# ZhengkunTian/OpenTransformer

Measured on AMD Instinct MI355X. Metric: utterances/sec (80-d fbank, ~1000 frames) train fwd+bwd, higher is better.
Workload: dtype fp16; 1 GPU; AISHELL-1 transformer_baseline.yaml (+input_size 80), 12 enc / 6 dec layers, B=32/GPU x 1000 frames x 80-d fbank, 15 decoder rows, V=4234, residual_dropout 0.1; step = fwd + bwd + grad all-reduce + clip/Adam/Noam; global_batch=32, frames=1000, parallelism=dp1, hipgraph=True

## Files before the change

include/otrans_hip.h:

```cpp
#ifndef OTRANS_HIP_H
#define OTRANS_HIP_H
#include <stddef.h>
#include <stdint.h>
#ifdef __cplusplus
extern "C" {
#endif

#define OTR_F32 0
#define OTR_BF16 1
#define OTR_F16 2
#define OTR_ACT_NONE 0
#define OTR_ACT_RELU 1

#define OTR_ABI_VERSION 604
int32_t otr_version(void);
int32_t otr_half_type(void);
int32_t otr_debug_set(int32_t key, int32_t value);
int32_t otr_set_fault_counter(void* device_word);
int32_t otr_debug_trread(const void* image, const int32_t* addr, void* out, void* stream);
int32_t otr_debug_trace(void* buf);
const char* otr_last_error_string(void);

typedef struct {
  int32_t M, N, K;
  int32_t x_dtype, w_dtype, y_dtype, compute;
  int64_t ldx, ldw, ldy;
  int32_t act;
  int32_t accumulate;
} otr_linear_desc_t;
int32_t otr_linear_fwd(const otr_linear_desc_t* d, const void* x, const void* w, const float* bias, void* y,
                       void* workspace, int64_t workspace_bytes, void* stream);
int32_t otr_linear_fwd_batched(const otr_linear_desc_t* d, const void* x, const void* w, void* y, int32_t nbatch, int64_t bsx, int64_t bsw,
                               int64_t bsy, void* stream);
int32_t otr_linear_dgrad(const otr_linear_desc_t* d, const void* dy, const void* w, void* dx, void* workspace,
                         int64_t workspace_bytes, void* stream);
int32_t otr_linear_wgrad(const otr_linear_desc_t* d, const void* dy, const void* x, void* dw, void* workspace,
                         int64_t workspace_bytes, void* stream);
int32_t otr_colsum(const void* a, int32_t dtype, int64_t M, int64_t N, int64_t lda, float* out, int32_t accumulate,
                   void* stream);

int32_t otr_ffn_glu_fwd(const void* x, int64_t ldx, const void* w1, int64_t ldw, const float* b1, void* h, void* u, int32_t M,
                        int32_t F, int32_t d_model, void* stream);
int32_t otr_ffn_glu_bwd(const void* dy, int32_t dy_dtype, int64_t ldy, const void* w2t, int64_t ldw, const void* h,
                        int32_t h_has_sigmoid, void* dh, float* dbias_partial, int32_t partial_rows_cap,
                        int32_t* partial_rows, int32_t M, int32_t F, int32_t d_model, void* stream);

int32_t otr_pack_frags(const void* src, void* dst, const int64_t* table, int32_t n_items, int64_t total_blocks,
// ... 221 lines not shown
int32_t otr_dwconv_bwd_part(const float* dy, const void* g, int32_t dtype, const float* w, void* dg, float* part, int32_t B, int32_t T,
                            int32_t C, int32_t k, int32_t pad, void* stream);
int32_t otr_bn_swish_fwd(const float* y, const float* stats, const float* gamma, const float* beta, float* running_mean,
                         float* running_var, float* saved, void* out, int32_t out_dtype, int64_t M, int32_t C, float eps,
                         float momentum, int32_t training, void* stream);
int64_t otr_dwconv_fwd_partial_rows(int64_t M);
int32_t otr_dwconv_fwd_part(const void* g, int32_t dtype, const float* w, const float* bias, float* y, float* spart, int32_t B, int32_t T,
                            int32_t C, int32_t k, int32_t pad, void* stream);
int32_t otr_bn_swish_fwd_part(const float* y, const float* spart, int32_t nblk, const float* gamma, const float* beta, float* running_mean,
                              float* running_var, float* saved, void* out, int32_t out_dtype, int64_t M, int32_t C, float eps,
                              float momentum, void* stream);
int32_t otr_bn_swish_bwd_partial_rows(int64_t M);
int32_t otr_bn_swish_bwd(const float* y, const void* ds, int32_t ds_dtype, const float* saved, const float* gamma,
                         const float* beta, float* red, float* partial, float* dgamma_acc, float* dbeta_acc, float* dy,
                         int64_t M, int32_t C, int32_t training, void* stream);
int32_t otr_bn_swish_bwd_sums(const float* y, const void* ds, int32_t ds_dtype, const float* saved, const float* gamma, const float* beta,
                              float* red, float* partial, float* dgamma_acc, float* dbeta_acc, int64_t M, int32_t C, void* stream);
int32_t otr_conformer_conv_bwd_mid(const float* y, const void* ds, const float* saved, const float* gamma, const float* beta,
                                   const float* red, const void* g, const float* w, const void* h, const uint8_t* row_mask, void* dh,
                                   float* part, float* gpart, int32_t dtype, int32_t training, int32_t B, int32_t T, int32_t C, int32_t k,
                                   int32_t pad, void* stream);

int32_t otr_ctc_loss(const float* log_probs, const int64_t* targets, int64_t ldt, const int32_t* in_len,
                     const int32_t* tgt_len, int32_t B, int32_t T, int32_t V, int32_t max_tgt, int32_t blank,
                     float* alpha_ws, float* nll, float* loss, float* dlogits, void* stream);

#define OTR_OPT_STATE_FLOATS 528
int32_t otr_optimizer_step(float* param, const float* grad, float* exp_avg, float* exp_avg_sq, int64_t n,
                           float* state, int32_t state_floats ,
                           void* param_bf16 ,
                           float base_lr, float beta1, float beta2, float eps, float weight_decay,
                           float grad_scale, float clip_norm, float noam_model_size, float noam_warmup,
                           float noam_factor, float noam_step_offset, float grad_noise_std, void* stream);

int32_t otr_allreduce_unique_id(void* id128);
int32_t otr_allreduce_init(void** handle, const void* id128, int32_t rank, int32_t world);
int32_t otr_allreduce_run(void* handle, void* buf, int64_t count, int32_t dtype, void* stream);
int32_t otr_allreduce_destroy(void* handle);

int32_t otr_beam_topk(const float* logits, int64_t ld, const float* lm_logits, int64_t ld_lm, float lm_weight,
                      int64_t rows, int32_t V, int32_t k, float* out_score, int64_t* out_idx, void* stream);
int32_t otr_beam_prune(const float* k_score, const int64_t* k_idx, const float* scores_in, const uint8_t* flag_in,
                       const int64_t* preds_in, int64_t ldp, int32_t batch, int32_t beam, int32_t t, int32_t eos,
                       float* scores_out, uint8_t* flag_out, int64_t* preds_out, int32_t* n_finished, void* stream);

int64_t otr_ctc_beam_workspace_bytes(int32_t B, int32_t T, int32_t W);
int32_t otr_ctc_topk(const float* log_probs, int64_t ld, const int32_t* lengths, int32_t B, int32_t T, int32_t V, int32_t K,
                     float* top_lp, int32_t* top_tok, void* stream);
int32_t otr_ctc_beam_search(const float* top_lp, const int32_t* top_tok, const int32_t* lengths, int32_t B, int32_t T, int32_t V,
                            int32_t K, int32_t blank, int32_t W, void* workspace, int64_t ws_bytes, int64_t* tokens,
                            int32_t* out_len, float* scores, void* stream);

int32_t otr_ngram_lookup(const void* table, int64_t capacity, int32_t max_probe, int32_t order, int32_t V, const int32_t* ctx,
                         const int32_t* ctx_len, const int32_t* tok, int64_t n, float oov_score, float* out, void* stream);
int32_t otr_ctc_beam_search_lm(const float* top_lp, const int32_t* top_tok, const int32_t* lengths, int32_t B, int32_t T, int32_t V,
                               int32_t K, int32_t blank, int32_t W, void* workspace, int64_t ws_bytes, int64_t* tokens,
                               int32_t* out_len, float* scores, const void* table, int64_t capacity, int32_t max_probe,
                               int32_t order, float alpha, float beta, float oov_score, float* lm_scores, void* stream);

int64_t otr_ctc_align_workspace_bytes(int32_t B, int32_t T, int32_t max_tgt);
int32_t otr_ctc_align(const float* log_probs, int64_t ld, const int64_t* targets, int64_t ldt, const int32_t* in_len,
                      const int32_t* tgt_len, int32_t B, int32_t T, int32_t V, int32_t max_tgt, int32_t blank, void* workspace,
                      int64_t ws_bytes, int32_t* frame_token, int32_t* spans, float* label_logp, float* score, void* stream);

int32_t otr_joint_prebeam(const float* logits, int64_t ld, const float* lm_logits, int64_t ld_lm, float att_weight, float lm_weight,
                          int64_t rows, int32_t V, int32_t K, float* cand_score, int32_t* cand_idx, void* stream);
// ... 111 lines not shown
```

opentransformer_amd/_lib.py:

```python
import ctypes as C
import os

_HERE = os.path.dirname(os.path.abspath(__file__))
_LIB_DIR = os.environ.get('OTR_LIB_DIR') or os.path.join(_HERE, 'lib')
LIB_PATHS = {'bf16': os.path.join(_LIB_DIR, 'libotrans_hip.so'), 'fp16': os.path.join(_LIB_DIR, 'libotrans_hip_f16.so')}
LIB_PATH = LIB_PATHS['bf16']

OTR_F32, OTR_BF16, OTR_F16 = 0, 1, 2
OTR_ABI_VERSION = 604
OTR_OPT_STATE_FLOATS = 528
ACT_NONE, ACT_RELU = 0, 1


class LinearDesc(C.Structure):
    _fields_ = [('M', C.c_int32), ('N', C.c_int32), ('K', C.c_int32),
                ('x_dtype', C.c_int32), ('w_dtype', C.c_int32), ('y_dtype', C.c_int32), ('compute', C.c_int32),
                ('ldx', C.c_int64), ('ldw', C.c_int64), ('ldy', C.c_int64),
                ('act', C.c_int32), ('accumulate', C.c_int32)]


class WgradItem(C.Structure):
    _fields_ = [('dy', C.c_void_p), ('x', C.c_void_p), ('dw', C.c_void_p), ('M', C.c_int32), ('N', C.c_int32),
                ('K', C.c_int32), ('ldy', C.c_int64), ('ldx', C.c_int64), ('ldw', C.c_int64),
                ('dy_dtype', C.c_int32), ('x_dtype', C.c_int32), ('dbias', C.c_void_p), ('overwrite', C.c_int32)]


class ColsumItem(C.Structure):
    _fields_ = [('a', C.c_void_p), ('out', C.c_void_p), ('M', C.c_int64), ('N', C.c_int64), ('lda', C.c_int64),
                ('dtype', C.c_int32)]


class AttnDesc(C.Structure):
    _fields_ = [('B', C.c_int32), ('H', C.c_int32), ('Tq', C.c_int32), ('Tk', C.c_int32), ('dk', C.c_int32),
                ('dtype', C.c_int32),
                ('q_bs', C.c_int64), ('q_ts', C.c_int64), ('k_bs', C.c_int64), ('k_ts', C.c_int64),
                ('v_bs', C.c_int64), ('v_ts', C.c_int64), ('o_bs', C.c_int64), ('o_ts', C.c_int64),
                ('causal', C.c_int32), ('scale', C.c_float)]


class LnDesc(C.Structure):
    _fields_ = [('M', C.c_int64), ('d', C.c_int32), ('a_dtype', C.c_int32),
                ('eps', C.c_float), ('p_drop', C.c_float), ('rng_offset', C.c_uint64), ('a_scale', C.c_float), ('a_row_mask', C.c_void_p),
# ... 111 lines not shown
    'otr_conv2_dgrad_wide': [C.POINTER(ConvDesc), _P, _P, _P, _P, _P, _I64, _P],
    'otr_debug_conv2_dgrad_plan': [C.POINTER(ConvDesc), _P],
    'otr_conv2_wgrad': [C.POINTER(ConvDesc), _P, _P, _P, _P, _I64, _P],
    'otr_relu_bwd': [_P, _P, _P, _I32, _I64, _P],
    'otr_relu_bwd_colsum_partial_rows': [_I64, _I32, _I32],
    'otr_relu_bwd_colsum': [_P, _P, _P, _P, _I32, _I64, _I32, _P],
    'otr_act_fwd': [_P, _P, _I32, _I64, _I32, _P],
    'otr_act_bwd': [_P, _P, _P, _I32, _I64, _I32, _P],
    'otr_label_smoothing_loss': [_P, _P, _I64, _I32, _F32, _I32, _P, _P, _P, _P],
    'otr_label_smoothing_loss_ld': [_P, _I64, _P, _I64, _I32, _F32, _I32, _P, _P, _I64, _P, _P],
    'otr_label_smoothing_loss_fused': [_P, _I64, _P, _I64, _I32, _I64, _I32, _F32, _I32, _P, _P, _P, _I32, _I64, _P, _P, _P],
    'otr_log_softmax': [_P, _P, _I64, _I32, _P],
    'otr_ctc_loss': [_P, _P, _I64, _P, _P, _I32, _I32, _I32, _I32, _I32, _P, _P, _P, _P, _P],
    'otr_ffn_fwd_split_slab': [_P, _P, _P, _P, _P, _P, _P, _I64, _I32, _I32, _P],
    'otr_ffn_bwd_split_slab': [_P, _P, _P, _P, _P, _P, _I64, _I32, _I32, _P],
    'otr_ln_bwd_proj_slabs': [_P, _P, _I32, _P, _P, _P, _P, _P, _P, _P, _P, _P, _I64, _P, _I64, _I32, _F32, C.c_uint64, _P],
    'otr_rb_linear_ln': [C.POINTER(DecLn), _P, _P, _P, _I32, _I64, _I64, _I32, _I32, _P],
    'otr_dec_self_fwd': [C.POINTER(DecLn), _I32, _I32, _P, _P, _P, _P, _P, _P, _P, _P],
    'otr_dec_self_step': [C.POINTER(DecLn), _I64, _P, _P, _P, _P, _P, _P, _P, _I32, _P, _P],
    'otr_dec_cross_fwd': [C.POINTER(DecLn), _I32, _I32, _P, _P, _P, _P, _I64, _I64, _I32, _I32, _P, _I32, _P, _P, _P, _P, _P],
    'otr_dec_cross_fwd_shared': [C.POINTER(DecLn), _I32, _I32, _P, _P, _P, _P, _I64, _I64, _I32, _I32, _P, _I32, _I32, _P, _P, _P, _P, _P],
    'otr_dec_ffn_hsave_bytes': [_I64, _I32],
    'otr_dec_ffn_fwd': [C.POINTER(DecLn), _I64, _P, _P, _P, _I32, _I32, _P, _P, _P],
    'otr_dec_ln': [C.POINTER(DecLn), _I64, _P],
    'otr_dec_self_step_pair': [C.POINTER(DecSelfStep), C.POINTER(DecSelfStep), _P],
    'otr_dec_ffn_fwd_pair': [C.POINTER(DecFfnFwd), C.POINTER(DecFfnFwd), _P],
    'otr_dec_ln_pair': [C.POINTER(DecLn), _I64, C.POINTER(DecLn), _I64, _P],
    'otr_dec_ffn_bwd': [C.POINTER(DecLnB), _I64, _P, _P, _P, _I32, _I32, _P, _P, _P, _P, _P],
    'otr_dec_cross_bwd': [C.POINTER(DecLnB), _I32, _I32, _P, _P, _P, _P, _P, _P, _P, _I64, _I64, _I32, _I32, _P, _I32, _P, _P, _P],
    'otr_dec_self_bwd': [C.POINTER(DecLnB), _I32, _I32, _P, _P, _P, _P, _P, _P, _P, _P],
    'otr_dec_sum': [_P, _P, _I32, _I64, _P, _P],
    'otr_dec_group_size': [_I32, _I32],
    'otr_optimizer_step': [_P, _P, _P, _P, _I64, _P, _I32, _P] + [_F32] * 12 + [_P],
    'otr_allreduce_unique_id': [_P],
    'otr_allreduce_init': [C.POINTER(C.c_void_p), _P, _I32, _I32],
    'otr_allreduce_run': [_P, _P, _I64, _I32, _P],
    'otr_allreduce_destroy': [_P],
    'otr_beam_topk': [_P, _I64, _P, _I64, _F32, _I64, _I32, _I32, _P, _P, _P],
    'otr_beam_prune': [_P, _P, _P, _P, _P, _I64, _I32, _I32, _I32, _I32, _P, _P, _P, _P, _P],
    'otr_beam_prune_cached': [_P, _P, _P, _P, _P, _I64, _I32, _I32, _I32, _P, _P, _P, _P, _I32, _P, _P, _P, _P, _P],
    'otr_ctc_beam_workspace_bytes': [_I32, _I32, _I32],
    'otr_ctc_topk': [_P, _I64, _P, _I32, _I32, _I32, _I32, _P, _P, _P],
    'otr_ctc_beam_search': [_P, _P, _P, _I32, _I32, _I32, _I32, _I32, _I32, _P, _I64, _P, _P, _P, _P],
    'otr_ngram_lookup': [_P, _I64, _I32, _I32, _I32, _P, _P, _P, _I64, _F32, _P, _P],
    'otr_ctc_beam_search_lm': [_P, _P, _P, _I32, _I32, _I32, _I32, _I32, _I32, _P, _I64, _P, _P, _P, _P, _I64, _I32, _I32, _F32, _F32,
                               _F32, _P, _P],
    'otr_ctc_align_workspace_bytes': [_I32, _I32, _I32],
    'otr_ctc_align': [_P, _I64, _P, _I64, _P, _P, _I32, _I32, _I32, _I32, _I32, _P, _I64, _P, _P, _P, _P, _P],
    'otr_joint_prebeam': [_P, _I64, _P, _I64, _F32, _F32, _I64, _I32, _I32, _P, _P, _P],
    'otr_ctc_prefix_score': [_P, _I64, _P, _I32, _I32, _I32, _I32, _I32, _I64, _I32, _I32, _P, _P, _P, _P, _I64, _I32, _P, _P, _P, _P, _P,
                             _F32, _P, _P, _P, _I32, _P, _P, _P, _P],
    'otr_beam_prune_joint': [_P, _P, _P, _P, _P, _I64, _I32, _I32, _I32, _I32, _P, _P, _P, _P, _P, _P, _P],
    'otr_beam_prune_cached_joint': [_P, _P, _P, _P, _P, _I64, _I32, _I32, _I32, _P, _P, _P, _P, _I32, _P, _P, _P, _P, _P, _P, _P],
    'otr_rescore_pack': [_P, _P, _P, _I64, _I32, _I32, _I32, _I32, _I32, _P, _P, _P, _P],
    'otr_rescore_score': [_P, _I64, _P, _I64, _P, _I64, _P, _I64, _I32, _I32, _P, _P, _P],
    'otr_rescore_select': [_P, _P, _P, _P, _P, _P, _I32, _I32, _I32, _I32, _F32, _F32, _F32, _F32, _P, _P, _P, _P, _P, _P],
    'otr_decode_embed': [_P, _I64, _P, _P, _P, _P, _I64, _I32, _I32, _F32, _P],
    'otr_decode_lookup': [_P, _I64, _P, _P, _P, _P, _I64, _I32, _I32, _P],
    'otr_lstm_cell': [_P, _P, _P, _P, _P, _P, _P, _I64, _I32, _P],
    'otr_lstm_step_supported': [_I64, _I32],
    'otr_lstm_pack_whh': [_P, _P, _P, _I32, _I32, _P],
    'otr_lstm_fwd_step': [_P, _P, _P, _P, _P, _P, _P, _P, _P, _I32, _I64, _I32, _P],
    'otr_lstm_bwd_step': [_P, _P, _P, _P, _P, _P, _P, _P, _P, _I32, _I64, _I32, _P],
    'otr_lstm_cell_fwd': [_P, _P, _P, _P, _P, _P, _P, _P, _I64, _I32, _P],
    'otr_lstm_cell_bwd': [_P, _P, _P, _P, _P, _P, _P, _P, _I32, _I64, _I32, _P],
    'otr_decode_self_attention': [_P, _P, _P, _P, _P, _P, _I32, _I64, _I32, _I32, _I32, _F32, _P],
# ... 76 lines not shown
```

opentransformer_amd/csrc/optim.hip:

```cpp
#include "common.h"

struct OptState {
  float step;
  float lr;
  float bc1, bc2;
  float sqnorm;
  float skipped;
  float loss_scale;
  float good_steps;
  float unscale;
  float growth_interval;
  float faults;
  float reserved[5];
  float norm_part[512];
};
constexpr int OPT_NORM_WG = 512;

__global__ void sqnorm_kernel(const float* g, int64_t n, OptState* st) {
  __shared__ float sh[4];
  float s = 0.f;
  const int64_t n4 = n / 4;
  const float4* g4 = reinterpret_cast<const float4*>(g);
  const int64_t stride = (int64_t)gridDim.x * blockDim.x;
  int64_t i = (int64_t)blockIdx.x * blockDim.x + threadIdx.x;
// ... 45 lines not shown
    if (st->growth_interval > 0.f && st->good_steps >= st->growth_interval) {
      st->loss_scale = fminf(ls * 2.f, 65536.f);
      st->good_steps = 0.f;
    }
  }
  float t = st->step + 1.f;
  st->step = t;
  st->bc1 = 1.f - powf(beta1, t);
  st->bc2 = 1.f - powf(beta2, t);
  if (warmup > 0.f) {
    float s = t + step_offset;
    st->lr = factor * rsqrtf(model_size) * fminf(rsqrtf(s), s * powf(warmup, -1.5f));
  } else {
    st->lr = base_lr;
  }
}

__device__ __forceinline__ float otr_gauss(uint64_t seed, uint64_t idx) {
  const float u1 = ((float)otr_rand32_sm64(seed, 2 * idx) + 1.f) * (1.f / 4294967296.f);
  const float u2 = (float)otr_rand32_sm64(seed, 2 * idx + 1) * (1.f / 4294967296.f);
  return sqrtf(-2.f * __logf(u1)) * __cosf(6.2831853f * u2);
}

__device__ __forceinline__ void adam_one(float& pi, float gi, float& mi, float& vi, int64_t i, float coef, float wd, float beta1, float beta2,
                                         float step_size, float rbc2, float eps, float noise_std, uint64_t nseed) {
  const bool pad = gi == 0.f && pi == 0.f;
  gi *= coef;
  if (noise_std > 0.f && !pad) gi += noise_std * otr_gauss(nseed, (uint64_t)i);
  gi += wd * pi;
  mi = beta1 * mi + (1.f - beta1) * gi;
  vi = beta2 * vi + (1.f - beta2) * gi * gi;
  pi = pi - step_size * mi / (sqrtf(vi) * rbc2 + eps);
}
__global__ __launch_bounds__(256) void adam_kernel(float* p, const float* g, float* m, float* v, int64_t n, const OptState* st, bf16_t* p_lp,
                                                   float beta1, float beta2, float eps, float wd, float clip, float noise_std) {
  const float us = st->unscale;
  const float norm = sqrtf(st->sqnorm) * us;
  if (!isfinite(norm)) return;
  const float coef = us * (clip > 0.f ? fminf(1.f, clip / (norm + 1e-6f)) : 1.f);
  const float lr = st->lr, bc1 = st->bc1, rbc2 = rsqrtf(st->bc2);
  const float step_size = lr / bc1;
  const uint64_t nseed = 0x6E015Eull + (uint64_t)st->step * 0x9E3779B97F4A7C15ull;
  typedef float f4 __attribute__((ext_vector_type(4)));
  const int64_t n4 = n >> 2;
  for (int64_t i = (int64_t)blockIdx.x * blockDim.x + threadIdx.x; i < n4; i += (int64_t)gridDim.x * blockDim.x) {
    f4 pv = __builtin_nontemporal_load(reinterpret_cast<const f4*>(p) + i);
    const f4 gv = *(reinterpret_cast<const f4*>(g) + i);
    f4 mv = __builtin_nontemporal_load(reinterpret_cast<const f4*>(m) + i);
    f4 vv = __builtin_nontemporal_load(reinterpret_cast<const f4*>(v) + i);
#pragma unroll
    for (int e = 0; e < 4; ++e) {
      float pi = pv[e], mi = mv[e], vi = vv[e];
      adam_one(pi, gv[e], mi, vi, 4 * i + e, coef, wd, beta1, beta2, step_size, rbc2, eps, noise_std, nseed);
      pv[e] = pi; mv[e] = mi; vv[e] = vi;
    }
    __builtin_nontemporal_store(mv, reinterpret_cast<f4*>(m) + i);
    __builtin_nontemporal_store(vv, reinterpret_cast<f4*>(v) + i);
    __builtin_nontemporal_store(pv, reinterpret_cast<f4*>(p) + i);
    if (p_lp) *reinterpret_cast<uint2*>(p_lp + 4 * i) = make_uint2((uint32_t)f2bf(pv[0]) | ((uint32_t)f2bf(pv[1]) << 16), (uint32_t)f2bf(pv[2]) | ((uint32_t)f2bf(pv[3]) << 16));
  }
  if (blockIdx.x == 0 && threadIdx.x < (n & 3)) {
    const int64_t i = 4 * n4 + threadIdx.x;
    float pi = p[i], mi = m[i], vi = v[i];
    adam_one(pi, g[i], mi, vi, i, coef, wd, beta1, beta2, step_size, rbc2, eps, noise_std, nseed);
    p[i] = pi; m[i] = mi; v[i] = vi;
    if (p_lp) p_lp[i] = f2bf(pi);
  }
}

extern "C" int32_t otr_optimizer_step(float* param, const float* grad, float* exp_avg, float* exp_avg_sq, int64_t n,
                                      float* state, int32_t state_floats, void* param_bf16, float base_lr, float beta1, float beta2, float eps,
                                      float weight_decay, float grad_scale, float clip_norm, float noam_model_size,
                                      float noam_warmup, float noam_factor, float noam_step_offset, float grad_noise_std,
                                      void* stream) {
  OTR_REQUIRE(param && grad && exp_avg && exp_avg_sq && state, "optimizer_step: null pointer");
  OTR_REQUIRE(n > 0, "optimizer_step: empty parameter buffer");
  OTR_REQUIRE(grad_noise_std >= 0.f, "optimizer_step: grad_noise_std must be >= 0");
  OTR_REQUIRE((uintptr_t)grad % 16 == 0, "optimizer_step: grad buffer must be 16-byte aligned");
  OTR_REQUIRE(state_floats >= OTR_OPT_STATE_FLOATS, "optimizer_step: the state block must hold OTR_OPT_STATE_FLOATS floats "
              "(the gradient-norm partial sums live behind the 16 state slots)");
  OTR_REQUIRE(((uintptr_t)param | (uintptr_t)exp_avg | (uintptr_t)exp_avg_sq) % 16 == 0 && (!param_bf16 || (uintptr_t)param_bf16 % 8 == 0),
              "optimizer_step: parameter / moment buffers must be 16-byte aligned (the 16-bit shadow 8-byte)");
  hipStream_t s = (hipStream_t)stream;
  OptState* st = reinterpret_cast<OptState*>(state);
  unsigned grid = (unsigned)((n / 4 + 255) / 256 > OPT_NORM_WG ? OPT_NORM_WG : (n / 4 + 255) / 256);
  if (grid < 1) grid = 1;
  hipLaunchKernelGGL(sqnorm_kernel, dim3(grid), dim3(256), 0, s, grad, n, st);
  hipLaunchKernelGGL(opt_tick_kernel, dim3(1), dim3(64), 0, s, st, base_lr, noam_model_size, noam_warmup, noam_factor,
                     noam_step_offset, beta1, beta2, grad_scale, g_otr_fault, (int)grid);
  unsigned g2 = (unsigned)((n / 4 + 255) / 256 > 4096 ? 4096 : (n / 4 + 255) / 256);
  if (g2 < 1) g2 = 1;
  hipLaunchKernelGGL(adam_kernel, dim3(g2), dim3(256), 0, s, param, grad, exp_avg, exp_avg_sq, n, st, (bf16_t*)param_bf16, beta1, beta2, eps,
                     weight_decay, clip_norm, grad_noise_std);
  return otr_check_launch("optimizer_step");
}
```

opentransformer_amd/dp.py:

```python
import contextlib
import ctypes as C
import dataclasses
import math

import torch
import torch.distributed as dist

from . import _lib as L
from . import ops

ALIGN = 64
_COMM_CODE = {torch.float32: L.OTR_F32, torch.bfloat16: L.OTR_BF16, torch.float16: L.OTR_F16}


def _align(n):
    return (n + ALIGN - 1) // ALIGN * ALIGN


def _rows8(rows):
    return (rows + 7) // 8 * 8


def _tiles(r, c):
    return ((r + 63) // 64) * ((c + 63) // 64)


def _spec(off, shape, stride=None):
    return (off, tuple(shape), tuple(stride or (math.prod(shape[k + 1:]) for k in range(len(shape)))))


def _view(buf, spec):
    return buf.as_strided(spec[1], spec[2], buf.storage_offset() + spec[0])


_VIEWS = {'pad': None, 'pad_lpt': 'flat_param_lpt', '_otr_regroup_grad': '_store_all', '_otr_lp_view': 'flat_param_lp',
          '_otr_lpt_view': 'flat_param_lpt', '_otr_regroup_view': 'flat_param_lpt', '_otr_ffn_packs': 'flat_pack',
          '_otr_lin_packs': 'flat_pack'}


@dataclasses.dataclass
class _Plan:
    offsets: list
    row_groups: list
    early_end: int
    numel: int
    lp: bool = False
    stage_total: int = 0
    lpt_table: list = dataclasses.field(default_factory=list)
    lpt_tiles: int = 0
    pack_table: list = dataclasses.field(default_factory=list)
    pack_blocks: int = 0
    pack_len: int = 0
    ffn_packed: list = dataclasses.field(default_factory=list)
    views: dict = dataclasses.field(default_factory=lambda: {name: {} for name in _VIEWS})


def _group_key(name, shape):
    for suffix in ('src_attn.vk_proj.weight', 'src_attn.vk_proj.bias'):
        if name.endswith(suffix) and math.prod(shape) % ALIGN == 0:
            return suffix, shape
    return None


def _slot_numel(shape):
    if len(shape) == 2 and shape[0] % 8 != 0 and shape[1] % 8 == 0 and shape[0] > 8:
        return _rows8(shape[0]) * shape[1]
    return math.prod(shape)


def _plan_flat(shapes, names, early):
    offs, total, row_groups, early_end = [None] * len(shapes), 0, [], 0
    for want_early in (True, False):
        todo = [i for i in range(len(shapes)) if early[i] == want_early]
        groups = {}
        for i in todo:
            groups.setdefault(_group_key(names[i], shapes[i]), []).append(i)
        for i in todo:
            if offs[i] is not None:
                continue
            k = _group_key(names[i], shapes[i])
            members = groups[k] if k is not None else [i]
            if len(members) > 1:
                row_groups.append(list(members))
            for j in members:
                offs[j] = total
                total += _align(_slot_numel(shapes[j]))
# ... 34 lines not shown

def _plan_transposed(plan, shapes, regrouped):
    lpt, pads, done = plan.views['_otr_lpt_view'], plan.views['pad'], set(plan.ffn_packed) | set(plan.views['_otr_lin_packs'])

    def transpose(off, rows, cols):
        plan.lpt_table.append([off, rows, cols, plan.lpt_tiles])
        plan.lpt_tiles += _tiles(rows, cols)
    for members in plan.row_groups:
        if len(shapes[members[0]]) != 2:
            continue
        rows, cols, o0 = sum(shapes[j][0] for j in members), shapes[members[0]][1], plan.offsets[members[0]]
        transpose(o0, rows, cols)
        for j in members:
            lpt[j] = _spec(o0, (cols, shapes[j][0]), (rows, 1))
            o0 += shapes[j][0]
        done.update(members)
    for i, (A, R, S), contiguous in regrouped:
        if i in done or math.prod(shapes[i]) != A * R * S or not contiguous:
            continue
        plan.views['_otr_regroup_view'][i] = _spec(plan.offsets[i], (A, S, R))
        for a in range(A):
            transpose(plan.offsets[i] + a * R * S, R, S)
        done.add(i)
    for i, (shape, off) in enumerate(zip(shapes, plan.offsets)):
        if i in done or len(shape) != 2:
            continue
        rows = pads[i][1][0] if i in pads else shape[0]
        lpt[i] = _spec(off, (shape[1], shape[0]), (rows, 1))
        if i in pads:
            plan.views['pad_lpt'][i] = _spec(off, (shape[1], rows))
        transpose(off, rows, shape[1])


def _plan(shapes, names, early, regrouped=(), ffn=(), *, cuda=False, fp32=True, half=False, flatten=True, rb_shapes=()):
    shapes = [tuple(s) for s in shapes]
    plan = _Plan(*_plan_flat(shapes, names, early), lp=flatten and cuda and fp32 and half)
    for i, s in enumerate(shapes if flatten and cuda else []):
        if (len(s) == 1 and s[0] % 8 != 0) or _slot_numel(s) != math.prod(s):
            plan.views['pad'][i] = _spec(plan.offsets[i], (_rows8(s[0]),) + s[1:])
    if cuda and fp32:
        _plan_stage(plan, shapes, regrouped)
    if plan.lp:
        plan.views['_otr_lp_view'] = {i: _spec(off, s) for i, (s, off) in enumerate(zip(shapes, plan.offsets))}
        _plan_packs(plan, shapes, ffn, rb_shapes)
        _plan_transposed(plan, shapes, regrouped)
    return plan


def _describe(module, params, early_modules=None):
    index = {id(p): i for i, p in enumerate(params)}
    name_of = {id(p): n for n, p in module.named_parameters()}
    early_ids = {id(p) for m in (early_modules or []) for p in m.parameters()}
    regrouped, ffn = [], []
    for mod in module.modules():
        regroup = getattr(mod, 'regrouped_weights', None)
        for p, ars in (regroup() if callable(regroup) else []):
            if id(p) in index:
                regrouped.append((index[id(p)], tuple(ars), p.is_contiguous()))
        w1, w2 = getattr(getattr(mod, 'w_1', None), 'weight', None), getattr(getattr(mod, 'w_2', None), 'weight', None)
        if getattr(mod, 'activation', None) == 'glu' and id(w1) in index and id(w2) in index:
            ffn.append((index[id(w1)], index[id(w2)]))
    return dict(shapes=[tuple(p.shape) for p in params], names=[name_of.get(id(p), '') for p in params],
                early=[id(p) in early_ids for p in params], regrouped=regrouped, ffn=ffn)


class FlatDataParallel:
    def __init__(self, module, process_group=None, flatten_params=True, comm='torch', grad_comm_dtype=None, early_modules=None):
        assert comm in ('torch', 'rccl')
        self.module, self.group = module, process_group
        self.comm, self.grad_comm_dtype = comm, grad_comm_dtype
        self._rccl = self._payload = self._side = None
        self._early_state = None
        self._accumulating = False
        self.skip_collectives = False
        self._single_writer = set()
        self.flat_param = self.flat_param_lp = self.flat_param_lpt = self.flat_pack = None
        self._lpt_table, self._lpt_tiles, self._pack_table, self._pack_blocks, self._ffn_packed = None, 0, None, 0, set()
        seen, self.params = set(), []
        for p in module.parameters():
            if p.requires_grad and id(p) not in seen:
                seen.add(id(p))
                self.params.append(p)
        dev, dt = self.params[0].device, self.params[0].dtype
        cuda = dev.type == 'cuda'
        self._plan = plan = _plan(**_describe(module, self.params, early_modules), cuda=cuda, fp32=dt == torch.float32,
                                  half=ops.is_half(), flatten=flatten_params, rb_shapes=ops._RB_SHAPES if ops._RB else ())
        self.offsets, self._row_groups, self.early_end, self.numel = plan.offsets, plan.row_groups, plan.early_end, plan.numel
        self.param_numel = sum(p.numel() for p in self.params)
        self._alloc_gradients(dev, dt)
        self._install_params(dev, dt, flatten_params)
        if cuda and flatten_params:
            self._register_single_writers()
        if plan.lp:
            self._install_shadows(dev)
            self._install_packs(dev)
            self._install_transposed(dev)
            self.refresh_lp()
        if cuda:
            ops.defer_weight_grads(True)
        if self.early_end > 0:
            ops.set_early_callback(self._on_early_mark, modules=list(module.modules()))

    def _install(self, *names):
        for name in names:
            buf = getattr(self, _VIEWS[name])
            for i, spec in self._plan.views[name].items():
                setattr(self.params[i], name, tuple(_view(buf, s) for s in spec) if name.endswith('packs') else _view(buf, spec))

    def _install_pad(self, key, buf, name='pad'):
        for i, spec in self._plan.views[name].items():
            self.params[i]._otr_pad[key] = _view(buf, spec)

    def _alloc_gradients(self, dev, dt):
        n = self.numel
        self._store_all = torch.zeros(n + ALIGN + self._plan.stage_total, device=dev, dtype=dt)
        self._grad_store = self._store_all[:n + ALIGN]
        self.flat_grad = self._grad_store[:n]
        self._fault_cell = self._grad_store[n:n + 1]
        self._install('_otr_regroup_grad')
        self._staged = [self.params[i] for i in sorted(self._plan.views['_otr_regroup_grad'])]
        for p in self._staged:
            p._otr_regroup_state = {'dirty': False}

    def _install_params(self, dev, dt, flatten_params):
        if flatten_params:
            self.flat_param = torch.empty(self.numel, device=dev, dtype=dt)
            self.flat_param.zero_()
        for p, off in zip(self.params, self.offsets):
            n = p.numel()
# ... 227 lines not shown

class FusedAdam:

    def __init__(self, dp, lr=1e-3, betas=(0.9, 0.98), eps=1e-9, weight_decay=1e-6, clip_grad=5.0,
                 noam=None, grad_noise=0.0, loss_scale=None, loss_scale_growth=2000):
        assert dp.flat_param is not None, 'FusedAdam needs FlatDataParallel(flatten_params=True)'
        self.dp = dp
        self.lr, self.betas, self.eps, self.wd, self.clip = lr, betas, eps, weight_decay, clip_grad
        self.noam = noam
        self.exp_avg = torch.zeros_like(dp.flat_param)
        self.exp_avg_sq = torch.zeros_like(dp.flat_param)
        self._state_store = torch.zeros(L.OTR_OPT_STATE_FLOATS, dtype=torch.float32, device=dp.flat_param.device)
        self.state = self._state_store[:16]
        self.grad_noise = float(grad_noise)
        self.step_offset = 2.0
        if dp.flat_param.is_cuda:
            ops.fault_counter(dp.flat_param.device)
            if loss_scale is None:
                loss_scale = 4096.0 if ops.get_compute_dtype() == 'fp16' else 0.0
            if loss_scale:
                self.state[6] = float(loss_scale)
                self.state[9] = float(loss_scale_growth)
                dp.module._otr_loss_scale = self.state[6:7]
            else:
                dp.module._otr_loss_scale = None

    def step(self, grad_scale=1.0):
        if not self.dp.flat_param.is_cuda:
            raise L.OtransHipError('FusedAdam runs on the GPU only')
        n = self.dp.flat_param.numel()
        nm = self.noam or {}
        ops.check_no_pending_stages('FusedAdam.step')
        self._last_grad_scale = float(grad_scale)
        ret = L.load().otr_optimizer_step(
            C.c_void_p(self.dp.flat_param.data_ptr()), C.c_void_p(self.dp.flat_grad.data_ptr()),
            C.c_void_p(self.exp_avg.data_ptr()), C.c_void_p(self.exp_avg_sq.data_ptr()), n,
            C.c_void_p(self.state.data_ptr()), self._state_store.numel(),
            C.c_void_p(self.dp.flat_param_lp.data_ptr()) if self.dp.flat_param_lp is not None else None,
            self.lr, self.betas[0], self.betas[1], self.eps, self.wd,
            grad_scale, self.clip, float(nm.get('model_size', 1.0)), float(nm.get('warmup_steps', 0.0)),
            float(nm.get('factor', 1.0)), self.step_offset,
            self.grad_noise,
            C.c_void_p(torch.cuda.current_stream().cuda_stream))
        L.check(ret, 'otr_optimizer_step')
        self.dp.refresh_transposed()

    @property
    def global_step(self):
        return int(self.state[0].item() + self.step_offset)

    def state_dict(self):
        st = self.state.tolist()
        state = {}
        for i, (p, off) in enumerate(zip(self.dp.params, self.dp.offsets)):
            n = p.numel()
            state[i] = {'step': torch.tensor(float(st[0])),
                        'exp_avg': self.exp_avg[off:off + n].view(p.shape).clone(),
                        'exp_avg_sq': self.exp_avg_sq[off:off + n].view(p.shape).clone()}
        group = {'lr': float(st[1]) if st[0] > 0 else self.lr, 'betas': tuple(self.betas), 'eps': self.eps, 'weight_decay': self.wd,
                 'amsgrad': False, 'maximize': False, 'foreach': None, 'capturable': False, 'differentiable': False, 'fused': None,
                 'params': list(range(len(self.dp.params)))}
        return {'state': state, 'param_groups': [group],
                'otr': {'state_block': self.state.detach().cpu().clone(), 'global_step': int(st[0] + self.step_offset)}}

    def load_state_dict(self, sd, global_step=None):
        state, groups = sd['state'], sd['param_groups']
        order = [i for g in groups for i in g['params']]
        if len(order) != len(self.dp.params):
            raise ValueError('optimizer checkpoint holds %d parameters, the model has %d' % (len(order), len(self.dp.params)))
        steps = set()
        self.exp_avg.zero_()
        self.exp_avg_sq.zero_()
        for key, p, off in zip(order, self.dp.params, self.dp.offsets):
            ent = state.get(key)
            if ent is None:
                continue
            n = p.numel()
            if tuple(ent['exp_avg'].shape) != tuple(p.shape):
# ... 30 lines not shown
```

opentransformer_amd/ops.py:

```python
import contextlib
import ctypes as C
import gc
import math

import torch

from . import _lib as L

_state = {'compute': 'bf16', 'rng_offset': 0, 'seed': None}


@contextlib.contextmanager
def graph_capture(graph, **kw):
    gc.collect()
    was_enabled = gc.isenabled()
    gc.disable()
    _capture['serial'] += 1
    _capture['active'] = _capture['serial']
    try:
        with torch.cuda.graph(graph, **kw):
            yield graph
    finally:
        _capture['active'] = None
        if was_enabled:
# ... 636 lines not shown
        _arm_flush()
        return out
    dw = out if out is not None else torch.empty((N, K), dtype=torch.float32, device=dy2.device)
    if out is not None:
        _wq_excl['written'].add(out.data_ptr())
    d = _linear_desc(M, N, K, x2.dtype, torch.float32, dy2.dtype, x2.stride(0), K, dy2.stride(0),
                     accumulate=int(out is not None))
    ws = _workspace(dy2.device)
    L.check(L.load().otr_linear_wgrad(C.byref(d), _p(dy2), _p(x2), _p(dw), _p(ws), _WS_BYTES, _stream()), 'otr_linear_wgrad')
    return dw


def colsum_raw(a2, out=None, defer=True):
    M, N = a2.shape
    acc = out is not None
    if acc and defer and _wq['on'] and a2.stride(1) == 1 and a2.data_ptr() % 16 == 0 and _in_backward():
        _wq['b'].append((a2, out))
        _arm_flush()
        return out
    if out is None:
        out = torch.empty((N,), dtype=torch.float32, device=a2.device)
    L.check(L.load().otr_colsum(_p(a2), _code(a2.dtype), M, N, a2.stride(0), _p(out), int(acc), _stream()), 'otr_colsum')
    return out


def _rows(x):
    x2 = x.reshape(-1, x.shape[-1])
    if x2.stride(1) != 1 or (x2.shape[0] > 1 and x2.stride(0) < x2.shape[1]):
        x2 = x2.contiguous()
    return x2


_RB = True
_RB_SHAPES = ((256, 256), (768, 256))
_RB_LINEAR_MIN_ROWS = 1024


def lin_pack_items(w_off, N, K, dst_off):
    return [[w_off, K, 1, N, K, 0, dst_off], [w_off, 1, K, K, N, 0, dst_off + N * K]], 2 * N * K


def lin_packs(w):
    if not _RB or _state['compute'] == 'fp32' or w is None or w.dim() != 2 or not w.is_cuda or tuple(w.shape) not in _RB_SHAPES:
        return None
    views = getattr(w, '_otr_lin_packs', None)
    if views is not None:
        return views
    if getattr(w, '_otr_grad_inplace', False):
        return None
    key = (w._version, w.data_ptr(), _state['compute'])
    cache = getattr(w, '_otr_lin_pack_cache', None)
    if cache is not None and cache[0] == key:
        return cache[1]
    N, K = w.shape
    src = weight_lp(w).reshape(-1)
    rows, total = lin_pack_items(0, N, K, 0)
    dst = torch.empty(total, dtype=src.dtype, device=src.device)
    pack_frags(src, dst, rows)
    packs = (dst[:N * K], dst[N * K:])
    w._otr_lin_pack_cache = (key, packs)
    return packs


def _rb_rows_ok(t2):
    return (t2 is not None and t2.dtype == half_dtype() and t2.dim() == 2 and t2.stride(1) == 1 and t2.stride(0) % 8 == 0
            and t2.data_ptr() % 16 == 0)
# ... 2669 lines not shown
```

Before: 8177 utterances/s.

## Fuse Adam update with transposed shadow and MFMA pack refresh per tile

Adds a tiled Adam kernel driven by a host-built table. For each 64x64 weight tile it performs the fp32 update, writes the 16-bit shadow, and stages it in shared memory to emit the transposed shadow and the packed operand layouts directly. Untiled regions are processed as flat chunks. This replaces the separate refresh_transposed pass, which reread the shadow to rebuild those layouts after every step. The cost is more complex indexing, a shared-memory stage, and a fallback to the old path whenever the planning constraints are not met.

```diff
diff --git a/include/otrans_hip.h b/include/otrans_hip.h
--- a/include/otrans_hip.h
+++ b/include/otrans_hip.h
@@ -12,7 +12,7 @@
 #define OTR_ACT_NONE 0
 #define OTR_ACT_RELU 1
 
-#define OTR_ABI_VERSION 604
+#define OTR_ABI_VERSION 605
 int32_t otr_version(void);
 int32_t otr_half_type(void);
 int32_t otr_debug_set(int32_t key, int32_t value);
@@ -300,6 +300,12 @@
                            float base_lr, float beta1, float beta2, float eps, float weight_decay,
                            float grad_scale, float clip_norm, float noam_model_size, float noam_warmup,
                            float noam_factor, float noam_step_offset, float grad_noise_std, void* stream);
+int32_t otr_optimizer_step_layouts(float* param, const float* grad, float* exp_avg, float* exp_avg_sq, int64_t n,
+                                   float* state, int32_t state_floats, void* param_16, void* param_16t, void* pack,
+                                   const int64_t* table, int32_t n_rows,
+                                   float base_lr, float beta1, float beta2, float eps, float weight_decay,
+                                   float grad_scale, float clip_norm, float noam_model_size, float noam_warmup,
+                                   float noam_factor, float noam_step_offset, float grad_noise_std, void* stream);
 
 int32_t otr_allreduce_unique_id(void* id128);
 int32_t otr_allreduce_init(void** handle, const void* id128, int32_t rank, int32_t world);
diff --git a/opentransformer_amd/_lib.py b/opentransformer_amd/_lib.py
--- a/opentransformer_amd/_lib.py
+++ b/opentransformer_amd/_lib.py
@@ -7,7 +7,7 @@
 LIB_PATH = LIB_PATHS['bf16']
 
 OTR_F32, OTR_BF16, OTR_F16 = 0, 1, 2
-OTR_ABI_VERSION = 604
+OTR_ABI_VERSION = 605
 OTR_OPT_STATE_FLOATS = 528
 ACT_NONE, ACT_RELU = 0, 1
 
@@ -185,6 +185,7 @@
     'otr_dec_sum': [_P, _P, _I32, _I64, _P, _P],
     'otr_dec_group_size': [_I32, _I32],
     'otr_optimizer_step': [_P, _P, _P, _P, _I64, _P, _I32, _P] + [_F32] * 12 + [_P],
+    'otr_optimizer_step_layouts': [_P, _P, _P, _P, _I64, _P, _I32, _P, _P, _P, _P, _I32] + [_F32] * 12 + [_P],
     'otr_allreduce_unique_id': [_P],
     'otr_allreduce_init': [C.POINTER(C.c_void_p), _P, _I32, _I32],
     'otr_allreduce_run': [_P, _P, _I64, _I32, _P],
diff --git a/opentransformer_amd/csrc/optim.hip b/opentransformer_amd/csrc/optim.hip
--- a/opentransformer_amd/csrc/optim.hip
+++ b/opentransformer_amd/csrc/optim.hip
@@ -101,47 +101,176 @@
   vi = beta2 * vi + (1.f - beta2) * gi * gi;
   pi = pi - step_size * mi / (sqrtf(vi) * rbc2 + eps);
 }
+struct AdamStep { float coef, step_size, rbc2; uint64_t nseed; };
+__device__ __forceinline__ bool adam_begin(const OptState* st, float clip, AdamStep& a) {
+  const float us = st->unscale;
+  const float norm = sqrtf(st->sqnorm) * us;
+  if (!isfinite(norm)) return false;
+  a.coef = us * (clip > 0.f ? fminf(1.f, clip / (norm + 1e-6f)) : 1.f);
+  const float lr = st->lr, bc1 = st->bc1;
+  a.rbc2 = rsqrtf(st->bc2);
+  a.step_size = lr / bc1;
+  a.nseed = 0x6E015Eull + (uint64_t)st->step * 0x9E3779B97F4A7C15ull;
+  return true;
+}
+__device__ __forceinline__ void adam_quad(f32x4& pv, const f32x4& gv, f32x4& mv, f32x4& vv, int64_t i0, const AdamStep& a, float wd, float beta1,
+                                          float beta2, float eps, float noise_std) {
+#pragma unroll
+  for (int e = 0; e < 4; ++e) {
+    float pi = pv[e], mi = mv[e], vi = vv[e];
+    adam_one(pi, gv[e], mi, vi, i0 + e, a.coef, wd, beta1, beta2, a.step_size, a.rbc2, eps, noise_std, a.nseed);
+    pv[e] = pi; mv[e] = mi; vv[e] = vi;
+  }
+}
+__device__ __forceinline__ uint2 adam_quad16(const f32x4& pv) {
+  return make_uint2((uint32_t)f2bf(pv[0]) | ((uint32_t)f2bf(pv[1]) << 16), (uint32_t)f2bf(pv[2]) | ((uint32_t)f2bf(pv[3]) << 16));
+}
+__device__ __forceinline__ bf16_t adam_scalar(float* p, const float* g, float* m, float* v, bf16_t* p_lp, int64_t i, const AdamStep& a, float wd,
+                                              float beta1, float beta2, float eps, float noise_std) {
+  float pi = p[i], mi = m[i], vi = v[i];
+  adam_one(pi, g[i], mi, vi, i, a.coef, wd, beta1, beta2, a.step_size, a.rbc2, eps, noise_std, a.nseed);
+  p[i] = pi; m[i] = mi; v[i] = vi;
+  const bf16_t h = f2bf(pi);
+  if (p_lp) p_lp[i] = h;
+  return h;
+}
 __global__ __launch_bounds__(256) void adam_kernel(float* p, const float* g, float* m, float* v, int64_t n, const OptState* st, bf16_t* p_lp,
                                                    float beta1, float beta2, float eps, float wd, float clip, float noise_std) {
-  const float us = st->unscale;
-  const float norm = sqrtf(st->sqnorm) * us;
-  if (!isfinite(norm)) return;
-  const float coef = us * (clip > 0.f ? fminf(1.f, clip / (norm + 1e-6f)) : 1.f);
-  const float lr = st->lr, bc1 = st->bc1, rbc2 = rsqrtf(st->bc2);
-  const float step_size = lr / bc1;
-  const uint64_t nseed = 0x6E015Eull + (uint64_t)st->step * 0x9E3779B97F4A7C15ull;
-  typedef float f4 __attribute__((ext_vector_type(4)));
+  AdamStep a;
+  if (!adam_begin(st, clip, a)) return;
   const int64_t n4 = n >> 2;
   for (int64_t i = (int64_t)blockIdx.x * blockDim.x + threadIdx.x; i < n4; i += (int64_t)gridDim.x * blockDim.x) {
-    f4 pv = __builtin_nontemporal_load(reinterpret_cast<const f4*>(p) + i);
-    const f4 gv = *(reinterpret_cast<const f4*>(g) + i);
-    f4 mv = __builtin_nontemporal_load(reinterpret_cast<const f4*>(m) + i);
-    f4 vv = __builtin_nontemporal_load(reinterpret_cast<const f4*>(v) + i);
-#pragma unroll
-    for (int e = 0; e < 4; ++e) {
-      float pi = pv[e], mi = mv[e], vi = vv[e];
-      adam_one(pi, gv[e], mi, vi, 4 * i + e, coef, wd, beta1, beta2, step_size, rbc2, eps, noise_std, nseed);
-      pv[e] = pi; mv[e] = mi; vv[e] = vi;
-    }
-    __builtin_nontemporal_store(mv, reinterpret_cast<f4*>(m) + i);
-    __builtin_nontemporal_store(vv, reinterpret_cast<f4*>(v) + i);
-    __builtin_nontemporal_store(pv, reinterpret_cast<f4*>(p) + i);
-    if (p_lp) *reinterpret_cast<uint2*>(p_lp + 4 * i) = make_uint2((uint32_t)f2bf(pv[0]) | ((uint32_t)f2bf(pv[1]) << 16), (uint32_t)f2bf(pv[2]) | ((uint32_t)f2bf(pv[3]) << 16));
-  }
-  if (blockIdx.x == 0 && threadIdx.x < (n & 3)) {
-    const int64_t i = 4 * n4 + threadIdx.x;
-    float pi = p[i], mi = m[i], vi = v[i];
-    adam_one(pi, g[i], mi, vi, i, coef, wd, beta1, beta2, step_size, rbc2, eps, noise_std, nseed);
-    p[i] = pi; m[i] = mi; v[i] = vi;
-    if (p_lp) p_lp[i] = f2bf(pi);
-  }
-}
-
-extern "C" int32_t otr_optimizer_step(float* param, const float* grad, float* exp_avg, float* exp_avg_sq, int64_t n,
-                                      float* state, int32_t state_floats, void* param_bf16, float base_lr, float beta1, float beta2, float eps,
-                                      float weight_decay, float grad_scale, float clip_norm, float noam_model_size,
-                                      float noam_warmup, float noam_factor, float noam_step_offset, float grad_noise_std,
-                                      void* stream) {
+    f32x4 pv = __builtin_nontemporal_load(reinterpret_cast<const f32x4*>(p) + i);
+    const f32x4 gv = *(reinterpret_cast<const f32x4*>(g) + i);
+    f32x4 mv = __builtin_nontemporal_load(reinterpret_cast<const f32x4*>(m) + i);
+    f32x4 vv = __builtin_nontemporal_load(reinterpret_cast<const f32x4*>(v) + i);
+    adam_quad(pv, gv, mv, vv, 4 * i, a, wd, beta1, beta2, eps, noise_std);
+    __builtin_nontemporal_store(mv, reinterpret_cast<f32x4*>(m) + i);
+    __builtin_nontemporal_store(vv, reinterpret_cast<f32x4*>(v) + i);
+    __builtin_nontemporal_store(pv, reinterpret_cast<f32x4*>(p) + i);
+    if (p_lp) *reinterpret_cast<uint2*>(p_lp + 4 * i) = adam_quad16(pv);
+  }
+  if (blockIdx.x == 0 && threadIdx.x < (n & 3))
+    adam_scalar(p, g, m, v, p_lp, 4 * n4 + threadIdx.x, a, wd, beta1, beta2, eps, noise_std);
+}
+
+constexpr int AL_PACK = 64 + 8;
+constexpr int AL_TR = 64 + 2;
+constexpr int AL_FLAT = 4096;
+__global__ __launch_bounds__(256) void adam_kernel_layouts(float* p, const float* g, float* m, float* v, const OptState* st, bf16_t* p_lp,
+                                                           bf16_t* p_lpt, bf16_t* pack, const int64_t* __restrict__ table, float beta1,
+                                                           float beta2, float eps, float wd, float clip, float noise_std) {
+  __shared__ __attribute__((aligned(16))) bf16_t tile[64 * AL_PACK];
+  AdamStep a;
+  if (!adam_begin(st, clip, a)) return;
+  const int64_t* t = table + (int64_t)blockIdx.x * 8;
+  const int64_t off = t[0], rows = t[1], cols = t[2], r0 = t[3], c0 = t[4], d0 = t[6], d1 = t[7];
+  const int flags = (int)t[5];
+  const int tid = threadIdx.x, lane = tid & 63, wid = tid >> 6, hi = lane >> 5;
+  if (flags & 16) {
+    const int64_t len = rows;
+    if (off % 4 == 0) {
+      const int64_t n4 = len >> 2;
+      for (int64_t k = tid; k < n4; k += 256) {
+        const int64_t i = (off >> 2) + k;
+        f32x4 pv = __builtin_nontemporal_load(reinterpret_cast<const f32x4*>(p) + i);
+        const f32x4 gv = *(reinterpret_cast<const f32x4*>(g) + i);
+        f32x4 mv = __builtin_nontemporal_load(reinterpret_cast<const f32x4*>(m) + i);
+        f32x4 vv = __builtin_nontemporal_load(reinterpret_cast<const f32x4*>(v) + i);
+        adam_quad(pv, gv, mv, vv, 4 * i, a, wd, beta1, beta2, eps, noise_std);
+        __builtin_nontemporal_store(mv, reinterpret_cast<f32x4*>(m) + i);
+        __builtin_nontemporal_store(vv, reinterpret_cast<f32x4*>(v) + i);
+        __builtin_nontemporal_store(pv, reinterpret_cast<f32x4*>(p) + i);
+        *reinterpret_cast<uint2*>(p_lp + 4 * i) = adam_quad16(pv);
+      }
+      if (tid < (len & 3)) adam_scalar(p, g, m, v, p_lp, off + 4 * n4 + tid, a, wd, beta1, beta2, eps, noise_std);
+    } else {
+      for (int64_t k = tid; k < len; k += 256) adam_scalar(p, g, m, v, p_lp, off + k, a, wd, beta1, beta2, eps, noise_std);
+    }
+    return;
+  }
+  const bool packs = (flags & 2) != 0;
+  const bool fast = r0 + 64 <= rows && c0 + 64 <= cols && cols % 8 == 0 && rows % 8 == 0 && off % 8 == 0;
+  if (!fast) {
+    const int h = (int)(rows - r0 < 64 ? rows - r0 : 64), w = (int)(cols - c0 < 64 ? cols - c0 : 64);
+    for (int e = tid; e < h * w; e += 256) {
+      const int r = e / w, c = e - r * w;
+      tile[r * AL_TR + c] = adam_scalar(p, g, m, v, p_lp, off + (r0 + r) * cols + c0 + c, a, wd, beta1, beta2, eps, noise_std);
+    }
+    if (!(flags & 1)) return;
+    __syncthreads();
+    for (int e = tid; e < h * w; e += 256) {
+      const int c = e / h, r = e - c * h;
+      p_lpt[off + (c0 + c) * rows + r0 + r] = tile[r * AL_TR + c];
+    }
+    return;
+  }
+  const int S = packs ? AL_PACK : AL_TR;
+  f32x4 pv[4], gv[4], mv[4], vv[4];
+  const int64_t base = off + r0 * cols + c0;
+  const uint32_t o0 = (uint32_t)(tid >> 4) * (uint32_t)cols + (tid & 15) * 4, ou = 16 * (uint32_t)cols;
+#pragma unroll
+  for (int u = 0; u < 4; ++u) {
+    const uint32_t o = o0 + u * ou;
+    pv[u] = __builtin_nontemporal_load(reinterpret_cast<const f32x4*>(p + base + o));
+    gv[u] = *reinterpret_cast<const f32x4*>(g + base + o);
+    mv[u] = __builtin_nontemporal_load(reinterpret_cast<const f32x4*>(m + base + o));
+    vv[u] = __builtin_nontemporal_load(reinterpret_cast<const f32x4*>(v + base + o));
+  }
+#pragma unroll
+  for (int u = 0; u < 4; ++u) {
+    const int id = tid + 256 * u, r = id >> 4, q = id & 15;
+    const uint32_t o = o0 + u * ou;
+    adam_quad(pv[u], gv[u], mv[u], vv[u], base + o, a, wd, beta1, beta2, eps, noise_std);
+    __builtin_nontemporal_store(mv[u], reinterpret_cast<f32x4*>(m + base + o));
+    __builtin_nontemporal_store(vv[u], reinterpret_cast<f32x4*>(v + base + o));
+    __builtin_nontemporal_store(pv[u], reinterpret_cast<f32x4*>(p + base + o));
+    const uint2 h = adam_quad16(pv[u]);
+    *reinterpret_cast<uint2*>(p_lp + base + o) = h;
+    uint32_t* row = reinterpret_cast<uint32_t*>(tile + r * S + q * 4);
+    row[0] = h.x; row[1] = h.y;
+  }
+  __syncthreads();
+  if (flags & 1) {
+    bf16_t* d = p_lpt + off;
+#pragma unroll
+    for (int u = 0; u < 2; ++u) {
+      const int id = tid + 256 * u, c = id >> 3, ch = id & 7;
+      uint32_t w[4];
+#pragma unroll
+      for (int e = 0; e < 4; ++e) w[e] = (uint32_t)tile[(ch * 8 + 2 * e) * S + c] | ((uint32_t)tile[(ch * 8 + 2 * e + 1) * S + c] << 16);
+      *reinterpret_cast<uint4*>(d + (c0 + c) * rows + r0 + ch * 8) = make_uint4(w[0], w[1], w[2], w[3]);
+    }
+  }
+  if (packs) {
+    const int perm0 = (flags >> 2) & 1, perm1 = (flags >> 3) & 1;
+#pragma unroll
+    for (int f2 = 0; f2 < 2; ++f2) {
+      const int f = wid * 2 + f2, rt = f >> 2, ks = f & 3;
+      const bf16_t* row = tile + (rt * 32 + (lane & 31)) * AL_PACK + ks * 16;
+      uint4 q;
+      if (perm0) {
+        const uint2 x = *reinterpret_cast<const uint2*>(row + 4 * hi), y = *reinterpret_cast<const uint2*>(row + 8 + 4 * hi);
+        q = make_uint4(x.x, x.y, y.x, y.y);
+      } else {
+        q = *reinterpret_cast<const uint4*>(row + 8 * hi);
+      }
+      *reinterpret_cast<uint4*>(pack + d0 + (((r0 >> 5) + rt) * (cols >> 4) + (c0 >> 4) + ks) * 512 + lane * 8) = q;
+      uint16_t e[8];
+#pragma unroll
+      for (int j = 0; j < 8; ++j) {
+        const int kk = perm1 ? (j < 4 ? 4 * hi + j : 8 + 4 * hi + (j - 4)) : hi * 8 + j;
+        e[j] = tile[(ks * 16 + kk) * AL_PACK + rt * 32 + (lane & 31)];
+      }
+      q = make_uint4(e[0] | ((uint32_t)e[1] << 16), e[2] | ((uint32_t)e[3] << 16), e[4] | ((uint32_t)e[5] << 16), e[6] | ((uint32_t)e[7] << 16));
+      *reinterpret_cast<uint4*>(pack + d1 + (((c0 >> 5) + rt) * (rows >> 4) + (r0 >> 4) + ks) * 512 + lane * 8) = q;
+    }
+  }
+}
+
+static int32_t opt_begin(float* param, const float* grad, float* exp_avg, float* exp_avg_sq, int64_t n, float* state, int32_t state_floats,
+                         void* param_bf16, float base_lr, float beta1, float beta2, float grad_scale, float noam_model_size, float noam_warmup,
+                         float noam_factor, float noam_step_offset, float grad_noise_std, hipStream_t s) {
   OTR_REQUIRE(param && grad && exp_avg && exp_avg_sq && state, "optimizer_step: null pointer");
   OTR_REQUIRE(n > 0, "optimizer_step: empty parameter buffer");
   OTR_REQUIRE(grad_noise_std >= 0.f, "optimizer_step: grad_noise_std must be >= 0");
@@ -150,16 +279,46 @@
               "(the gradient-norm partial sums live behind the 16 state slots)");
   OTR_REQUIRE(((uintptr_t)param | (uintptr_t)exp_avg | (uintptr_t)exp_avg_sq) % 16 == 0 && (!param_bf16 || (uintptr_t)param_bf16 % 8 == 0),
               "optimizer_step: parameter / moment buffers must be 16-byte aligned (the 16-bit shadow 8-byte)");
-  hipStream_t s = (hipStream_t)stream;
   OptState* st = reinterpret_cast<OptState*>(state);
   unsigned grid = (unsigned)((n / 4 + 255) / 256 > OPT_NORM_WG ? OPT_NORM_WG : (n / 4 + 255) / 256);
   if (grid < 1) grid = 1;
   hipLaunchKernelGGL(sqnorm_kernel, dim3(grid), dim3(256), 0, s, grad, n, st);
   hipLaunchKernelGGL(opt_tick_kernel, dim3(1), dim3(64), 0, s, st, base_lr, noam_model_size, noam_warmup, noam_factor,
                      noam_step_offset, beta1, beta2, grad_scale, g_otr_fault, (int)grid);
+  return 0;
+}
+
+extern "C" int32_t otr_optimizer_step(float* param, const float* grad, float* exp_avg, float* exp_avg_sq, int64_t n,
+                                      float* state, int32_t state_floats, void* param_bf16, float base_lr, float beta1, float beta2, float eps,
+                                      float weight_decay, float grad_scale, float clip_norm, float noam_model_size,
+                                      float noam_warmup, float noam_factor, float noam_step_offset, float grad_noise_std,
+                                      void* stream) {
+  hipStream_t s = (hipStream_t)stream;
+  if (int32_t e = opt_begin(param, grad, exp_avg, exp_avg_sq, n, state, state_floats, param_bf16, base_lr, beta1, beta2, grad_scale,
+                            noam_model_size, noam_warmup, noam_factor, noam_step_offset, grad_noise_std, s))
+    return e;
   unsigned g2 = (unsigned)((n / 4 + 255) / 256 > 4096 ? 4096 : (n / 4 + 255) / 256);
   if (g2 < 1) g2 = 1;
-  hipLaunchKernelGGL(adam_kernel, dim3(g2), dim3(256), 0, s, param, grad, exp_avg, exp_avg_sq, n, st, (bf16_t*)param_bf16, beta1, beta2, eps,
+  hipLaunchKernelGGL(adam_kernel, dim3(g2), dim3(256), 0, s, param, grad, exp_avg, exp_avg_sq, n, reinterpret_cast<const OptState*>(state),
+                     (bf16_t*)param_bf16, beta1, beta2, eps, weight_decay, clip_norm, grad_noise_std);
+  return otr_check_launch("optimizer_step");
+}
+
+extern "C" int32_t otr_optimizer_step_layouts(float* param, const float* grad, float* exp_avg, float* exp_avg_sq, int64_t n,
+                                              float* state, int32_t state_floats, void* param_16, void* param_16t, void* pack,
+                                              const int64_t* table, int32_t n_rows, float base_lr, float beta1, float beta2, float eps,
+                                              float weight_decay, float grad_scale, float clip_norm, float noam_model_size,
+                                              float noam_warmup, float noam_factor, float noam_step_offset, float grad_noise_std,
+                                              void* stream) {
+  OTR_REQUIRE(param_16 && table && n_rows > 0, "optimizer_step_layouts: the 16-bit shadow and a table with at least one row are required");
+  OTR_REQUIRE(((uintptr_t)param_16 | (uintptr_t)param_16t | (uintptr_t)pack) % 16 == 0,
+              "optimizer_step_layouts: the 16-bit shadow, its transposed form and the pack buffer must be 16-byte aligned");
+  hipStream_t s = (hipStream_t)stream;
+  if (int32_t e = opt_begin(param, grad, exp_avg, exp_avg_sq, n, state, state_floats, param_16, base_lr, beta1, beta2, grad_scale,
+                            noam_model_size, noam_warmup, noam_factor, noam_step_offset, grad_noise_std, s))
+    return e;
+  hipLaunchKernelGGL(adam_kernel_layouts, dim3((unsigned)n_rows), dim3(256), 0, s, param, grad, exp_avg, exp_avg_sq,
+                     reinterpret_cast<const OptState*>(state), (bf16_t*)param_16, (bf16_t*)param_16t, (bf16_t*)pack, table, beta1, beta2, eps,
                      weight_decay, clip_norm, grad_noise_std);
-  return otr_check_launch("optimizer_step");
-}
+  return otr_check_launch("optimizer_step_layouts");
+}
diff --git a/opentransformer_amd/dp.py b/opentransformer_amd/dp.py
--- a/opentransformer_amd/dp.py
+++ b/opentransformer_amd/dp.py
@@ -52,6 +52,7 @@
     pack_blocks: int = 0
     pack_len: int = 0
     ffn_packed: list = dataclasses.field(default_factory=list)
+    adam_table: list = None
     views: dict = dataclasses.field(default_factory=lambda: {name: {} for name in _VIEWS})
 
 
@@ -152,6 +153,42 @@
         transpose(off, rows, shape[1])
 
 
+ADAM_FLAT = 4096
+
+
+def _plan_adam(plan):
+    if not plan.lp:
+        return None
+    mats = {off: [rows, cols, 1, 0, 0] for off, rows, cols, _ in plan.lpt_table}
+    if len(mats) != len(plan.lpt_table):
+        return None
+    for src, rs, cs, rows, cols, perm, dst, _ in plan.pack_table:
+        straight = cs == 1 and rs == cols
+        R, C = (rows, cols) if straight else (cols, rows)
+        if not (straight or (rs == 1 and cs == C)) or R % 64 or C % 64 or src % 8 or dst % 8 or perm not in (0, 1):
+            return None
+        m = mats.setdefault(src, [R, C, 2, None, None])
+        if m[:2] != [R, C] or not m[2] & 2 or m[3 if straight else 4] is not None:
+            return None
+        m[3 if straight else 4] = dst
+        m[2] |= perm << (2 if straight else 3)
+    rows, pos = [], 0
+
+    def flat(lo, hi):
+        rows.extend([a, min(ADAM_FLAT, hi - a), 0, 0, 0, 16, 0, 0] for a in range(lo, hi, ADAM_FLAT))
+    for off in sorted(mats):
+        R, C, flags, d0, d1 = mats[off]
+        if off < pos or d0 is None or d1 is None:
+            return None
+        flat(pos, off)
+        rows.extend([off, R, C, r0, c0, flags, d0, d1] for r0 in range(0, R, 64) for c0 in range(0, C, 64))
+        pos = off + R * C
+    if pos > plan.numel:
+        return None
+    flat(pos, plan.numel)
+    return rows
+
+
 def _plan(shapes, names, early, regrouped=(), ffn=(), *, cuda=False, fp32=True, half=False, flatten=True, rb_shapes=()):
     shapes = [tuple(s) for s in shapes]
     plan = _Plan(*_plan_flat(shapes, names, early), lp=flatten and cuda and fp32 and half)
@@ -164,6 +201,7 @@
         plan.views['_otr_lp_view'] = {i: _spec(off, s) for i, (s, off) in enumerate(zip(shapes, plan.offsets))}
         _plan_packs(plan, shapes, ffn, rb_shapes)
         _plan_transposed(plan, shapes, regrouped)
+        plan.adam_table = _plan_adam(plan)
     return plan
 
 
@@ -196,6 +234,7 @@
         self._single_writer = set()
         self.flat_param = self.flat_param_lp = self.flat_param_lpt = self.flat_pack = None
         self._lpt_table, self._lpt_tiles, self._pack_table, self._pack_blocks, self._ffn_packed = None, 0, None, 0, set()
+        self._adam_table = None
         seen, self.params = set(), []
         for p in module.parameters():
             if p.requires_grad and id(p) not in seen:
@@ -215,6 +254,8 @@
             self._install_shadows(dev)
             self._install_packs(dev)
             self._install_transposed(dev)
+            if plan.adam_table:
+                self._adam_table = torch.tensor(plan.adam_table, dtype=torch.int64, device=dev)
             self.refresh_lp()
         if cuda:
             ops.defer_weight_grads(True)
@@ -508,18 +549,22 @@
         nm = self.noam or {}
         ops.check_no_pending_stages('FusedAdam.step')
         self._last_grad_scale = float(grad_scale)
-        ret = L.load().otr_optimizer_step(
-            C.c_void_p(self.dp.flat_param.data_ptr()), C.c_void_p(self.dp.flat_grad.data_ptr()),
-            C.c_void_p(self.exp_avg.data_ptr()), C.c_void_p(self.exp_avg_sq.data_ptr()), n,
-            C.c_void_p(self.state.data_ptr()), self._state_store.numel(),
-            C.c_void_p(self.dp.flat_param_lp.data_ptr()) if self.dp.flat_param_lp is not None else None,
-            self.lr, self.betas[0], self.betas[1], self.eps, self.wd,
-            grad_scale, self.clip, float(nm.get('model_size', 1.0)), float(nm.get('warmup_steps', 0.0)),
-            float(nm.get('factor', 1.0)), self.step_offset,
-            self.grad_noise,
-            C.c_void_p(torch.cuda.current_stream().cuda_stream))
-        L.check(ret, 'otr_optimizer_step')
-        self.dp.refresh_transposed()
+        def ptr(t):
+            return C.c_void_p(t.data_ptr()) if t is not None else None
+        dp = self.dp
+        head = (ptr(dp.flat_param), ptr(dp.flat_grad), ptr(self.exp_avg), ptr(self.exp_avg_sq), n,
+                ptr(self.state), self._state_store.numel(), ptr(dp.flat_param_lp))
+        tail = (self.lr, self.betas[0], self.betas[1], self.eps, self.wd,
+                grad_scale, self.clip, float(nm.get('model_size', 1.0)), float(nm.get('warmup_steps', 0.0)),
+                float(nm.get('factor', 1.0)), self.step_offset,
+                self.grad_noise,
+                C.c_void_p(torch.cuda.current_stream().cuda_stream))
+        if ops._ADAM_LAYOUTS and dp._adam_table is not None:
+            L.check(L.load().otr_optimizer_step_layouts(*head, ptr(dp.flat_param_lpt), ptr(dp.flat_pack), ptr(dp._adam_table),
+                                                        dp._adam_table.shape[0], *tail), 'otr_optimizer_step_layouts')
+        else:
+            L.check(L.load().otr_optimizer_step(*head, *tail), 'otr_optimizer_step')
+            dp.refresh_transposed()
 
     @property
     def global_step(self):
diff --git a/opentransformer_amd/ops.py b/opentransformer_amd/ops.py
--- a/opentransformer_amd/ops.py
+++ b/opentransformer_amd/ops.py
@@ -692,6 +692,7 @@
 
 
 _RB = True
+_ADAM_LAYOUTS = True
 _RB_SHAPES = ((256, 256), (768, 256))
 _RB_LINEAR_MIN_ROWS = 1024
 
```

Measured after the change: 8238 utterances/s (median of 6 runs). No clear change (+0.7%).
